# Weepingchestnut/SAVSR

Hardware: NVIDIA B200
Metric: hr_mpix_per_s (higher is better)
Workload: dtype bf16

## Files before the change

savsr_b200/csrc/conv_igemm.cu:

```cuda
#include <cstdio>
#include <cstdlib>

#include "common.cuh"

namespace savsr {

#ifdef SAVSR_DEBUG_COUNTERS
#define DBG_CLOCK() clock64()
#define DBG_ONLY(...) __VA_ARGS__
#else
#define DBG_CLOCK() 0ll
#define DBG_ONLY(...)
#endif

constexpr int kMaxAStages = 4;
constexpr int kHaloPitch = 10;
constexpr int kHaloStageBytes = 23552;
constexpr int kARegionBytes = 3 * kHaloStageBytes;
constexpr int kBBlocks = 18;
constexpr int kRing = 3;
constexpr int kEpiWarps = 8;
constexpr int kNumThreads = 64 + 32 * kEpiWarps;

struct ConvParams {
// ... 70 lines not shown
    if (c.res1_slot >= 0 && c.valid) {
      const uint4* r = reinterpret_cast<const uint4*>(p.arena + ((static_cast<long>(c.res1_slot) * p.batch + n) * npix + c.pix) * kC + col0);
#pragma unroll
      for (int j = 0; j < NC / 8; ++j) c.r1[j] = r[j];
    }
    if (c.res2_slot >= 0 && c.valid) {
      const uint4* r = reinterpret_cast<const uint4*>(p.arena + ((static_cast<long>(c.res2_slot) * p.batch + n) * npix + c.pix) * kC + col0);
#pragma unroll
      for (int j = 0; j < NC / 8; ++j) c.r2[j] = r[j];
    }
  }
}

__device__ __forceinline__ void add_h16x8(float* v, const uint4& u, float s, int fmt) {
  v[0] += s * h_lo(u.x, fmt); v[1] += s * h_hi(u.x, fmt); v[2] += s * h_lo(u.y, fmt); v[3] += s * h_hi(u.y, fmt);
  v[4] += s * h_lo(u.z, fmt); v[5] += s * h_hi(u.z, fmt); v[6] += s * h_lo(u.w, fmt); v[7] += s * h_hi(u.w, fmt);
}

template <int NC>
__device__ __forceinline__ void epi_finish(const ConvParams& p, const savsr_conv_group& g, int n, int tile, int quad, int lane,
                                           float (&v)[NC], int col0, const EpiCtx<NC>& c) {
  const long npix = static_cast<long>(p.height) * p.width;
  const float ns = c.neg_slope;
#pragma unroll
  for (int j = 0; j < NC; ++j) {
    const float t = v[j] + c.bias[j];
    v[j] = fmaxf(t, ns * t);
  }
  if constexpr (NC == 32) {
    if (c.has_mask) {
#pragma unroll
      for (int j = 0; j < NC; ++j) v[j] *= c.mk;
    }
    if (c.res1_slot >= 0 && c.valid) {
#pragma unroll
      for (int j = 0; j < NC / 8; ++j) add_h16x8(v + 8 * j, c.r1[j], 1.f, p.fmt);
    }
    if (c.res2_slot >= 0 && c.valid) {
      const float r2s = c.res2_scale;
#pragma unroll
      for (int j = 0; j < NC / 8; ++j) add_h16x8(v + 8 * j, c.r2[j], r2s, p.fmt);
    }
    if (c.valid) {
      uint4* d = reinterpret_cast<uint4*>(p.arena + ((static_cast<long>(c.dst_slot) * p.batch + n) * npix + c.pix) * kC + col0);
#pragma unroll
      for (int j = 0; j < NC / 8; ++j) {
        uint4 u;
        u.x = pack_h2(v[8 * j + 0], v[8 * j + 1], p.fmt);
        u.y = pack_h2(v[8 * j + 2], v[8 * j + 3], p.fmt);
        u.z = pack_h2(v[8 * j + 4], v[8 * j + 5], p.fmt);
        u.w = pack_h2(v[8 * j + 6], v[8 * j + 7], p.fmt);
        d[j] = u;
      }
    }
    if (c.pool != nullptr) {
      if (!c.valid) {
#pragma unroll
        for (int j = 0; j < NC; ++j) v[j] = 0.f;
      }
#pragma unroll
      for (int off = 16, cnt = 16; off >= 1; off >>= 1, cnt >>= 1) {
        const bool upper = (lane & off) != 0;
#pragma unroll
        for (int i = 0; i < cnt; ++i) {
          const float send = upper ? v[i] : v[i + cnt];
          const float keep = upper ? v[i + cnt] : v[i];
          v[i] = keep + __shfl_xor_sync(0xffffffffu, send, off);
        }
      }
      const int npart = p.tiles_x * p.tiles_y * 4;
      c.pool[(static_cast<long>(n) * npart + tile * 4 + quad) * kC + col0 + lane] = v[0];
    }
  } else {
    if (c.valid) {
      float4* d = reinterpret_cast<float4*>(static_cast<float*>(g.aux_dst) + (n * npix + c.pix) * 16);
#pragma unroll
      for (int j = 0; j < 4; ++j) d[j] = make_float4(v[4 * j], v[4 * j + 1], v[4 * j + 2], v[4 * j + 3]);
    }
  }
}


struct EpiQuad {
  float bias[8];
  uint4 r1[4], r2[4];
  float mk[4];
  long pix0;
  uint32_t valid;
  int bias_group;
  float neg_slope, res2_scale;
  int res1_slot, res2_slot, dst_slot;
  bool has_mask;
  float* pool;
  float psum[8];
};

__device__ __forceinline__ void epiq_prefetch(const ConvParams& p, const savsr_conv_group& g, int gi, int n, int tile, int quad,
                                              int lane, int half, EpiQuad& c) {
  const int tx = tile % p.tiles_x, ty = tile / p.tiles_x;
  const int px = tx * kTileW + (lane >> 2);
  const int py0 = ty * kTileH + quad * 4;
  const int rows = p.height - py0;
  c.valid = (px < p.width && rows > 0) ? (rows >= 4 ? 0xfu : ((1u << rows) - 1u)) : 0u;
  const long npix = static_cast<long>(p.height) * p.width;
  c.pix0 = static_cast<long>(py0) * p.width + px;
  const int ch0 = half * 32 + (lane & 3) * 8;
  if (gi != c.bias_group) {
    c.bias_group = gi;
    c.neg_slope = g.act == SAVSR_ACT_NONE ? 1.f : (g.act == SAVSR_ACT_RELU ? 0.f : g.slope);
    c.res2_scale = g.res2_scale;
    c.res1_slot = g.res1_slot; c.res2_slot = g.res2_slot; c.dst_slot = g.dst_slot;
    c.has_mask = g.mask != nullptr;
    c.pool = g.pool;
    if (g.bias != nullptr) {
      const float4 b0 = __ldg(reinterpret_cast<const float4*>(g.bias + ch0));
      const float4 b1 = __ldg(reinterpret_cast<const float4*>(g.bias + ch0) + 1);
      c.bias[0] = b0.x; c.bias[1] = b0.y; c.bias[2] = b0.z; c.bias[3] = b0.w;
      c.bias[4] = b1.x; c.bias[5] = b1.y; c.bias[6] = b1.z; c.bias[7] = b1.w;
    } else {
#pragma unroll
      for (int j = 0; j < 8; ++j) c.bias[j] = 0.f;
    }
  }
  if (c.has_mask) {
#pragma unroll
    for (int j = 0; j < 4; ++j) c.mk[j] = ((c.valid >> j) & 1u) ? __ldg(g.mask + n * npix + c.pix0 + j * p.width) : 0.f;
  }
  if (c.res1_slot >= 0) {
    const __nv_bfloat16* r = p.arena + ((static_cast<long>(c.res1_slot) * p.batch + n) * npix + c.pix0) * kC + ch0;
#pragma unroll
    for (int j = 0; j < 4; ++j)
      if ((c.valid >> j) & 1u) c.r1[j] = *reinterpret_cast<const uint4*>(r + static_cast<long>(j) * p.width * kC);
  }
  if (c.res2_slot >= 0) {
    const __nv_bfloat16* r = p.arena + ((static_cast<long>(c.res2_slot) * p.batch + n) * npix + c.pix0) * kC + ch0;
#pragma unroll
    for (int j = 0; j < 4; ++j)
      if ((c.valid >> j) & 1u) c.r2[j] = *reinterpret_cast<const uint4*>(r + static_cast<long>(j) * p.width * kC);
  }
}

template <class Release, class Next>
__device__ __forceinline__ void epiq_finish(const ConvParams& p, int n, int tile, int quad, int lane, int half, uint32_t taddr,
                                            EpiQuad& c, bool last_of_run, Release release, Next next) {
  uint32_t ra[16], rb[16];
  tmem_ld_16x256b_x4(taddr, ra);
  tmem_ld_16x256b_x4(taddr + (16u << 16), rb);
  tmem_ld_wait();
  tc_fence_before();
  __syncwarp();
  release();
  float v[4][8];
#pragma unroll
  for (int k = 0; k < 4; ++k) {
#pragma unroll
    for (int e = 0; e < 4; ++e) {
      v[e >> 1][2 * k + (e & 1)] = __uint_as_float(ra[4 * k + e]);
      v[2 + (e >> 1)][2 * k + (e & 1)] = __uint_as_float(rb[4 * k + e]);
    }
  }
  const long npix = static_cast<long>(p.height) * p.width;
  const int ch0 = half * 32 + (lane & 3) * 8;
  const float ns = c.neg_slope;
#pragma unroll
  for (int j = 0; j < 4; ++j) {
#pragma unroll
    for (int i = 0; i < 8; ++i) {
      const float t = v[j][i] + c.bias[i];
      v[j][i] = fmaxf(t, ns * t);
    }
  }
  if (c.has_mask) {
#pragma unroll
    for (int j = 0; j < 4; ++j) {
#pragma unroll
      for (int i = 0; i < 8; ++i) v[j][i] *= c.mk[j];
    }
  }
  if (c.res1_slot >= 0) {
#pragma unroll
    for (int j = 0; j < 4; ++j)
      if ((c.valid >> j) & 1u) add_h16x8(v[j], c.r1[j], 1.f, p.fmt);
  }
  if (c.res2_slot >= 0) {
    const float r2s = c.res2_scale;
#pragma unroll
    for (int j = 0; j < 4; ++j)
      if ((c.valid >> j) & 1u) add_h16x8(v[j], c.r2[j], r2s, p.fmt);
  }
  const uint32_t valid = c.valid;
  float* const pool = c.pool;
  __nv_bfloat16* d = p.arena + ((static_cast<long>(c.dst_slot) * p.batch + n) * npix + c.pix0) * kC + ch0;
  next();
#pragma unroll
  for (int j = 0; j < 4; ++j) {
    if ((valid >> j) & 1u) {
      uint4 u;
      u.x = pack_h2(v[j][0], v[j][1], p.fmt);
      u.y = pack_h2(v[j][2], v[j][3], p.fmt);
      u.z = pack_h2(v[j][4], v[j][5], p.fmt);
      u.w = pack_h2(v[j][6], v[j][7], p.fmt);
      *reinterpret_cast<uint4*>(d + static_cast<long>(j) * p.width * kC) = u;
    }
  }
  if (pool != nullptr) {
    if (valid == 0xfu) {
#pragma unroll
      for (int i = 0; i < 8; ++i) c.psum[i] += (v[0][i] + v[1][i]) + (v[2][i] + v[3][i]);
    } else {
#pragma unroll
      for (int i = 0; i < 8; ++i) {
        const float a0 = (valid & 1u) ? v[0][i] : 0.f, a1 = (valid & 2u) ? v[1][i] : 0.f;
        const float a2 = (valid & 4u) ? v[2][i] : 0.f, a3 = (valid & 8u) ? v[3][i] : 0.f;
        c.psum[i] += (a0 + a1) + (a2 + a3);
      }
    }
    const int npart = p.tiles_x * p.tiles_y * 4;
    const int ch = ch0 + ((lane >> 4) & 1) * 4 + ((lane >> 3) & 1) * 2 + ((lane >> 2) & 1);
    float total = 0.f;
    if (last_of_run) {
      float s[8];
#pragma unroll
      for (int i = 0; i < 8; ++i) { s[i] = c.psum[i]; c.psum[i] = 0.f; }
#pragma unroll
      for (int off = 16, cnt = 4; off >= 4; off >>= 1, cnt >>= 1) {
        const bool upper = (lane & off) != 0;
#pragma unroll
        for (int i = 0; i < cnt; ++i) {
          const float send = upper ? s[i] : s[i + cnt];
          const float keep = upper ? s[i + cnt] : s[i];
          s[i] = keep + __shfl_xor_sync(0xffffffffu, send, off);
        }
      }
      total = s[0];
    }
    pool[(static_cast<long>(n) * npart + tile * 4 + quad) * kC + ch] = total;
  }
}

__device__ __forceinline__ constexpr uint32_t desc_hi(uint32_t sbo_bytes) { return (sbo_bytes >> 4) | (1u << 14) | (2u << 29); }
__device__ __forceinline__ uint64_t make_desc(uint32_t hi, uint32_t lo) { return (static_cast<uint64_t>(hi) << 32) | lo; }

template <int BN, int KS, bool HALO>
__global__ void __launch_bounds__(kNumThreads, 1) conv_igemm_kernel(const __grid_constant__ ConvParams p) {
  constexpr int NT = KS * KS;
  extern __shared__ uint8_t smem_raw[];
  uint8_t* smem = reinterpret_cast<uint8_t*>((reinterpret_cast<uintptr_t>(smem_raw) + 1023) & ~static_cast<uintptr_t>(1023));
  constexpr int kBBytes = BN * 128;
  constexpr int kAStage = HALO ? kHaloStageBytes : kTileM * 128;
  constexpr int kAStages = HALO ? 3 : 4;
  uint8_t* smem_a = smem;
  uint8_t* smem_b = smem + kARegionBytes;
  uint8_t* smem_ring = smem_b + (kBBlocks - kRing) * kBBytes;
  uint64_t* bars = reinterpret_cast<uint64_t*>(smem_b + kBBlocks * kBBytes);
  uint64_t* a_full = bars;
  uint64_t* a_empty = a_full + kMaxAStages;
  uint64_t* res_full = a_empty + kMaxAStages;
  uint64_t* ring_full = res_full + kBBlocks;
  uint64_t* ring_empty = ring_full + kRing;
  uint64_t* res_free = ring_empty + kRing;
  uint64_t* t_full = res_free + 1;
  uint64_t* t_empty = t_full + 2;
  uint32_t* tmem_slot = reinterpret_cast<uint32_t*>(t_empty + 2);

  const int warp = threadIdx.x >> 5;
  const int lane = threadIdx.x & 31;
  const int tiles = p.tiles_x * p.tiles_y;
  const int total = p.ngroups * p.batch * tiles;
  const int item_begin = blockIdx.x * p.chunk;
  const int item_end = min(item_begin + p.chunk, total);
  const int nsrc = p.nsrc;
  const int n_res = p.n_res;
  constexpr int kTmemCols = 2 * BN < 32 ? 32 : 2 * BN;
  constexpr int kEpiArrivals = BN == 64 ? 8 : 4;

  if (warp == 0 && lane == 0) {
    prefetch_tensormap(HALO ? &p.tm_halo : &p.tm_tile);
    for (int i = 0; i < kMaxAStages; ++i) { mbar_init(a_full + i, 1); mbar_init(a_empty + i, 1); }
    for (int i = 0; i < kBBlocks; ++i) mbar_init(res_full + i, 1);
    for (int i = 0; i < kRing; ++i) { mbar_init(ring_full + i, 1); mbar_init(ring_empty + i, 1); }
    mbar_init(res_free, 1);
    for (int i = 0; i < 2; ++i) { mbar_init(t_full + i, 1); mbar_init(t_empty + i, kEpiArrivals); }
    fence_barrier_init();
  }
  if (warp == 1) tmem_alloc<kTmemCols>(tmem_slot);
  tc_fence_before();
  __syncthreads();
  tc_fence_after();
  const uint32_t tmem_base = *tmem_slot;

  if (warp == 0) {
    if (lane == 0) {
      int sa = 0, pa = 0, sr = 0, pr = 0;
      int gen = -1, cur_key = -1;
      long long dbg_ae = 0;
      const int nkb = nsrc * NT;
      int tile = item_begin % tiles;
      int gn = item_begin / tiles;
      for (int item = item_begin; item < item_end; ++item) {
        const int n = gn % p.batch;
        const int gi = gn / p.batch;
        const savsr_conv_group& g = p.g[gi];
        const int ty = tile / p.tiles_x;
        const int x0 = (tile - ty * p.tiles_x) * kTileW, y0 = ty * kTileH;
        const uint8_t* wptr = static_cast<const uint8_t*>(g.weight) + static_cast<long>(n) * g.weight_sample_stride;
        const int key = gi * p.batch + (g.weight_sample_stride != 0 ? n : 0);
        if (key != cur_key) {
          if (gen >= 0) mbar_wait(res_free, gen & 1);
          ++gen;
          cur_key = key;
          int kb = blockIdx.x % nkb;
          for (int i = 0; i < nkb; ++i) {
            if (kb < n_res) {
              mbar_expect_tx(res_full + kb, kBBytes);
              bulk_load(smem_b + kb * kBBytes, wptr + static_cast<long>(kb) * kBBytes, kBBytes, res_full + kb);
            }
            if (++kb == nkb) kb = 0;
          }
        }
        for (int s = 0; s < nsrc; ++s) {
// ... 79 lines not shown
#pragma unroll
              for (int k = 0; k < 4; ++k)
                umma_bf16(d_tmem, make_desc(a_hi, al + 2 * k), make_desc(b_hi, bl + 2 * k), idesc, (s | tap | k) ? 1u : 0u);
            }
            umma_commit(a_empty + sa);
          }
          __syncwarp();
          b_lo += NT * (kBBytes >> 4);
          if (++sa == kAStages) { sa = 0; pa ^= 1; }
        }
      } else {
        uint32_t accumulate = 0;
        uint32_t b_lo = b_lo0;
        int kb = 0;
        for (int s = 0; s < nsrc; ++s) {
          if constexpr (HALO) {
            mbar_wait(a_full + sa, pa);
            tc_fence_after();
          }
#pragma unroll
          for (int tap = 0; tap < NT; ++tap, ++kb, b_lo += kBBytes >> 4) {
            if constexpr (!HALO) {
              mbar_wait(a_full + sa, pa);
              tc_fence_after();
            }
            uint32_t bl = b_lo;
            const bool streamed = kb >= n_res;
            if (streamed) {
              mbar_wait(ring_full + sr, pr);
              tc_fence_after();
              bl = ring_lo0 + sr * (kBBytes >> 4);
            } else if (fresh) {
              mbar_wait(res_full + kb, gen & 1);
              tc_fence_after();
            }
            const uint32_t al = a_lo0 + sa * (kAStage >> 4) + (HALO ? ((tap / 3) * kHaloPitch + tap % 3) * 8 : 0);
            if (elect_one()) {
#pragma unroll
              for (int k = 0; k < 4; ++k) {
                umma_bf16(d_tmem, make_desc(a_hi, al + 2 * k), make_desc(b_hi, bl + 2 * k), idesc, accumulate);
                accumulate = 1;
              }
              if (streamed) umma_commit(ring_empty + sr);
              if (!HALO) umma_commit(a_empty + sa);
            }
            __syncwarp();
            accumulate = 1;
            if (streamed) {
              if (++sr == kRing) { sr = 0; pr ^= 1; }
            }
            if constexpr (!HALO) {
              if (++sa == kAStages) { sa = 0; pa ^= 1; }
            }
          }
          if constexpr (HALO) {
            if (elect_one()) umma_commit(a_empty + sa);
            __syncwarp();
            if (++sa == kAStages) { sa = 0; pa ^= 1; }
          }
        }
      }
      if (elect_one()) umma_commit(t_full + acc);
      __syncwarp();
      if (++tile == tiles) {
        tile = 0;
        if (++n == batch) { n = 0; ++gi; }
      }
    }
    DBG_ONLY(if (p.dbg != nullptr && lane == 0) {
      p.dbg[blockIdx.x * 8 + 0] = DBG_CLOCK() - dbg_t0;
      p.dbg[blockIdx.x * 8 + 1] = dbg_te;
      p.dbg[blockIdx.x * 8 + 2] = dbg_af;
      p.dbg[blockIdx.x * 8 + 3] = item_end - item_begin;
    })
    (void)dbg_te; (void)dbg_af; (void)dbg_t0;
  } else {
    const int quad = warp & 3;
    const int half = (warp - 2) >> 2;
    if (BN == 64 || half == 0) {
      constexpr int NC = 16;
      EpiCtx<NC> ec;
      EpiQuad eq;
      ec.bias_group = -1;
      eq.bias_group = -1;
#pragma unroll
      for (int i = 0; i < 8; ++i) eq.psum[i] = 0.f;
      int it = 0;
      int tile = item_begin % tiles;
      int gn = item_begin / tiles;
      long long dbg_tf = 0, dbg_t0 = DBG_CLOCK();
      if constexpr (BN == 64) {
        if (item_begin < item_end) epiq_prefetch(p, p.g[gn / p.batch], gn / p.batch, gn % p.batch, tile, quad, lane, half, eq);
      }
      for (int item = item_begin; item < item_end; ++item, ++it) {
        const int n = gn % p.batch;
        const int gi = gn / p.batch;
        const savsr_conv_group& g = p.g[gi];
        const int acc = it & 1;
        if constexpr (BN != 64) epi_prefetch<NC>(p, g, gi, n, tile, quad, lane, 0, ec);
        const long long c0 = DBG_CLOCK();
        mbar_wait(t_full + acc, (it >> 1) & 1);
        dbg_tf += DBG_CLOCK() - c0;
        tc_fence_after();
        const uint32_t taddr = tmem_base + (static_cast<uint32_t>(quad * 32) << 16) + static_cast<uint32_t>(acc * BN + half * 32);
        if constexpr (BN == 64) {
          epiq_finish(p, n, tile, quad, lane, half, taddr, eq, item + 1 >= item_end || tile + 1 == tiles,
                      [&] { if (lane == 0) mbar_arrive(t_empty + acc); }, [&] {
            if (item + 1 < item_end) {
              const int nt = tile + 1 == tiles ? 0 : tile + 1, ngn = tile + 1 == tiles ? gn + 1 : gn;
              epiq_prefetch(p, p.g[ngn / p.batch], ngn / p.batch, ngn % p.batch, nt, quad, lane, half, eq);
            }
          });
        } else {
          float v[NC];
          uint32_t r[16];
          tmem_ld16(taddr, r);
          tmem_ld_wait();
#pragma unroll
          for (int c = 0; c < 16; ++c) v[c] = __uint_as_float(r[c]);
          tc_fence_before();
          __syncwarp();
          if (lane == 0) mbar_arrive(t_empty + acc);
          epi_finish<NC>(p, g, n, tile, quad, lane, v, 0, ec);
        }
        if (++tile == tiles) { tile = 0; ++gn; }
      }
      DBG_ONLY(if (p.dbg != nullptr && warp == 2 && lane == 0) {
        p.dbg[blockIdx.x * 8 + 4] = DBG_CLOCK() - dbg_t0;
        p.dbg[blockIdx.x * 8 + 5] = dbg_tf;
      })
      (void)dbg_tf; (void)dbg_t0;
    }
  }

  tc_fence_before();
  __syncthreads();
  if (warp == 1) {
    tc_fence_after();
    tmem_dealloc<kTmemCols>(tmem_base);
  }
}

constexpr int kBatchTiles = 4;

constexpr int kBigkThreads = kNumThreads + 32;

__global__ void __launch_bounds__(kBigkThreads, 1) conv_igemm_bigk_kernel(const __grid_constant__ ConvParams p) {
  constexpr int BN = 64, NT = 9;
  constexpr int kBBytes = BN * 128;
  constexpr int kAStage = kHaloStageBytes, kAStages = 3;
  constexpr int kSetBlocks = 9, kSetBytes = kSetBlocks * kBBytes;
  extern __shared__ uint8_t smem_raw[];
  uint8_t* smem = reinterpret_cast<uint8_t*>((reinterpret_cast<uintptr_t>(smem_raw) + 1023) & ~static_cast<uintptr_t>(1023));
  uint8_t* smem_a = smem;
  uint8_t* smem_b = smem + kARegionBytes;
  uint64_t* bars = reinterpret_cast<uint64_t*>(smem_b + 2 * kSetBytes);
  uint64_t* a_full = bars;
  uint64_t* a_empty = a_full + kMaxAStages;
  uint64_t* set_full = a_empty + kMaxAStages;
  uint64_t* set_empty = set_full + 2;
  uint64_t* t_full = set_empty + 2;
  uint64_t* t_empty = t_full + 2 * kBatchTiles;
  uint32_t* tmem_slot = reinterpret_cast<uint32_t*>(t_empty + 2 * kBatchTiles);

  const int warp = threadIdx.x >> 5;
  const int lane = threadIdx.x & 31;
  const int tiles = p.tiles_x * p.tiles_y;
  const int total = p.ngroups * p.batch * tiles;
  const int item_begin = blockIdx.x * p.chunk;
  const int item_end = min(item_begin + p.chunk, total);
  const int nsrc = p.nsrc;
  const bool pinned = nsrc <= 2;
  const uint32_t ps_mask = p.per_sample_mask;

  if (warp == 0 && lane == 0) {
    prefetch_tensormap(&p.tm_halo);
    for (int i = 0; i < kMaxAStages; ++i) { mbar_init(a_full + i, 1); mbar_init(a_empty + i, p.issuers); }
    for (int i = 0; i < 2; ++i) { mbar_init(set_full + i, 1); mbar_init(set_empty + i, p.issuers); }
    for (int i = 0; i < 2 * kBatchTiles; ++i) { mbar_init(t_full + i, 1); mbar_init(t_empty + i, 8); }
    fence_barrier_init();
  }
  if (warp == 1) tmem_alloc<512>(tmem_slot);
  tc_fence_before();
  __syncthreads();
  tc_fence_after();
  const uint32_t tmem_base = *tmem_slot;
  pdl_wait();
  pdl_trigger();

  int item = item_begin;
  int tile = item_begin % tiles;
  int gn = item_begin / tiles;
  int bcount = 0;
  uint32_t use_bits = 0;
  uint32_t set_loads[2] = {0, 0};
  int cur_key = -1;

  if (warp == 0) {
    if (lane == 0) {
      int sa = 0, pa = 0;
      uint32_t u = 0;
      while (item < item_end) {
        const int cnt = min(kBatchTiles, min(item_end - item, tiles - tile));
        const int n = gn % p.batch;
        const int gi = gn / p.batch;
        const savsr_conv_group& g = p.g[gi];
        const uint8_t* wptr = static_cast<const uint8_t*>(g.weight) + static_cast<long>(n) * g.weight_sample_stride;
        const int key = gi * p.batch + (((ps_mask >> gi) & 1u) ? n : 0);
        const bool load = !pinned || key != cur_key;
        cur_key = key;
        for (int s = 0; s < nsrc; ++s) {
          if (load) {
            const int set = pinned ? s : static_cast<int>(u++ & 1);
            mbar_wait(set_empty + set, (set_loads[set] & 1u) ^ 1u);
            ++set_loads[set];
            mbar_expect_tx(set_full + set, kSetBytes);
            int kb = blockIdx.x % kSetBlocks;
            for (int i = 0; i < kSetBlocks; ++i) {
              bulk_load(smem_b + set * kSetBytes + kb * kBBytes, wptr + static_cast<long>(s * NT + kb) * kBBytes, kBBytes, set_full + set);
              if (++kb == kSetBlocks) kb = 0;
            }
          }
          const int img = g.src_slot[s] * p.batch + n;
          for (int j = 0; j < cnt; ++j) {
            const int tj = tile + j;
            const int ty = tj / p.tiles_x;
            mbar_wait(a_empty + sa, pa ^ 1);
            mbar_expect_tx(a_full + sa, kHaloPitch * (kTileH + 2) * 128u);
            tma_load_4d(smem_a + sa * kAStage, &p.tm_halo, a_full + sa, 0, (tj - ty * p.tiles_x) * kTileW - 1, ty * kTileH - 1, img);
            if (++sa == kAStages) { sa = 0; pa ^= 1; }
          }
        }
        item += cnt; tile += cnt;
        if (tile == tiles) { tile = 0; ++gn; }
      }
    }
  } else if (warp == 1 || (warp == 10 && p.issuers == 2)) {
    const int my = warp == 1 ? 0 : 1;
    const int own_mask = p.issuers == 2 ? 1 : 0;
    const uint32_t idesc = umma_idesc_f16(BN, p.fmt);
    constexpr uint32_t a_hi = desc_hi(kHaloPitch * 128u);
    constexpr uint32_t b_hi = desc_hi(1024u);
    const uint32_t a_lo0 = (smem_u32(smem_a) >> 4) & 0x3fffu;
    const uint32_t b_lo0 = (smem_u32(smem_b) >> 4) & 0x3fffu;
    int sa = 0, pa = 0;
    uint32_t u = 0;
    long long dbg_te = 0, dbg_af = 0, dbg_sf = 0, dbg_t0 = DBG_CLOCK(), c0;
    while (item < item_end) {
      const int cnt = min(kBatchTiles, min(item_end - item, tiles - tile));
      const int bb = bcount & 1;
      const int n = gn % p.batch;
      const int gi = gn / p.batch;
      const int key = gi * p.batch + (((ps_mask >> gi) & 1u) ? n : 0);
      const bool load = !pinned || key != cur_key;
      if (pinned && load && cur_key >= 0) {
        if (elect_one()) {
          for (int s = 0; s < nsrc; ++s) umma_commit(set_empty + s);
        }
        __syncwarp();
      }
      cur_key = key;
      c0 = DBG_CLOCK();
#pragma unroll
      for (int j = 0; j < kBatchTiles; ++j) {
// ... 4 lines not shown
      for (int s = 0; s < nsrc; ++s) {
        const int set = pinned ? s : static_cast<int>(u & 1);
        if (load) {
          c0 = DBG_CLOCK();
          mbar_wait(set_full + set, set_loads[set] & 1u);
          dbg_sf += DBG_CLOCK() - c0;
          ++set_loads[set];
          tc_fence_after();
          ++u;
        }
        const uint32_t bl0 = b_lo0 + set * (kSetBytes >> 4);
#pragma unroll
        for (int j = 0; j < kBatchTiles; ++j) {
          if (j < cnt) {
            c0 = DBG_CLOCK();
            mbar_wait(a_full + sa, pa);
            dbg_af += DBG_CLOCK() - c0;
            if ((j & own_mask) != my) {
              if (elect_one()) mbar_arrive(a_empty + sa);
              __syncwarp();
            } else {
              tc_fence_after();
              const uint32_t al0 = a_lo0 + sa * (kAStage >> 4);
              const uint32_t d_tmem = tmem_base + static_cast<uint32_t>((bb * kBatchTiles + j) * BN);
              if (elect_one()) {
                uint32_t al = al0, bl = bl0, acc = s ? 1u : 0u;
                if (p.ksteps == 4) {
#pragma unroll 1
                  for (int dy = 0; dy < 3; ++dy) {
#pragma unroll
                    for (int dx = 0; dx < 3; ++dx) {
#pragma unroll
                      for (int k = 0; k < 4; ++k) {
                        umma_bf16(d_tmem, make_desc(a_hi, al + dx * 8 + 2 * k), make_desc(b_hi, bl + dx * (kBBytes >> 4) + 2 * k), idesc, acc);
                        acc = 1u;
                      }
                    }
                    al += kHaloPitch * 8;
                    bl += 3 * (kBBytes >> 4);
                  }
                } else {
#pragma unroll 1
                  for (int dy = 0; dy < 3; ++dy) {
#pragma unroll
                    for (int dx = 0; dx < 3; ++dx) {
#pragma unroll 1
                      for (int k = 0; k < p.ksteps; ++k) {
                        umma_bf16(d_tmem, make_desc(a_hi, al + dx * 8 + 2 * k), make_desc(b_hi, bl + dx * (kBBytes >> 4) + 2 * k), idesc, acc);
                        acc = 1u;
                      }
                    }
                    al += kHaloPitch * 8;
                    bl += 3 * (kBBytes >> 4);
                  }
                }
                umma_commit(a_empty + sa);
                if (s == nsrc - 1) umma_commit(t_full + bb * kBatchTiles + j);
              }
              __syncwarp();
            }
            if (++sa == kAStages) { sa = 0; pa ^= 1; }
          }
        }
        if (!pinned) {
          if (elect_one()) umma_commit(set_empty + set);
          __syncwarp();
        }
      }
#pragma unroll
      for (int j = 0; j < kBatchTiles; ++j)
        if (j < cnt) use_bits ^= 1u << (bb * kBatchTiles + j);
      ++bcount;
      item += cnt; tile += cnt;
      if (tile == tiles) { tile = 0; ++gn; }
    }
    DBG_ONLY(if (p.dbg != nullptr && lane == 0 && my == 0) {
      p.dbg[blockIdx.x * 8 + 0] = DBG_CLOCK() - dbg_t0;
      p.dbg[blockIdx.x * 8 + 1] = dbg_te;
      p.dbg[blockIdx.x * 8 + 2] = dbg_af;
      p.dbg[blockIdx.x * 8 + 3] = item_end - item_begin;
      p.dbg[blockIdx.x * 8 + 7] = dbg_sf;
    })
    (void)dbg_te; (void)dbg_af; (void)dbg_sf; (void)dbg_t0;
  } else if (warp < 10) {
    const int quad = warp & 3;
    const int half = (warp - 2) >> 2;
    EpiQuad eq;
    eq.bias_group = -1;
#pragma unroll
    for (int i = 0; i < 8; ++i) eq.psum[i] = 0.f;
    long long dbg_tf = 0, dbg_t0 = DBG_CLOCK();
    if (item < item_end) epiq_prefetch(p, p.g[gn / p.batch], gn / p.batch, gn % p.batch, tile, quad, lane, half, eq);
    while (item < item_end) {
      const int cnt = min(kBatchTiles, min(item_end - item, tiles - tile));
      const int bb = bcount & 1;
      const int n = gn % p.batch;
      for (int j = 0; j < cnt; ++j) {
        const int acc = bb * kBatchTiles + j;
        const long long c0 = DBG_CLOCK();
        mbar_wait(t_full + acc, (use_bits >> acc) & 1u);
        dbg_tf += DBG_CLOCK() - c0;
        use_bits ^= 1u << acc;
        tc_fence_after();
        const uint32_t taddr = tmem_base + (static_cast<uint32_t>(quad * 32) << 16) + static_cast<uint32_t>(acc * BN + half * 32);
        epiq_finish(p, n, tile + j, quad, lane, half, taddr, eq, item + j + 1 >= item_end || tile + j + 1 == tiles,
                    [&] { if (lane == 0) mbar_arrive(t_empty + acc); }, [&] {
          if (item + j + 1 < item_end) {
            const int nt = tile + j + 1 == tiles ? 0 : tile + j + 1, ngn = tile + j + 1 == tiles ? gn + 1 : gn;
            epiq_prefetch(p, p.g[ngn / p.batch], ngn / p.batch, ngn % p.batch, nt, quad, lane, half, eq);
          }
        });
      }
      ++bcount;
      item += cnt; tile += cnt;
      if (tile == tiles) { tile = 0; ++gn; }
    }
    DBG_ONLY(if (p.dbg != nullptr && warp == 2 && lane == 0) {
      p.dbg[blockIdx.x * 8 + 4] = DBG_CLOCK() - dbg_t0;
      p.dbg[blockIdx.x * 8 + 5] = dbg_tf;
    })
    (void)dbg_tf; (void)dbg_t0;
  }

  tc_fence_before();
  __syncthreads();
  if (warp == 1) {
    tc_fence_after();
    tmem_dealloc<512>(tmem_base);
  }
}

template <int BN>
__global__ void __launch_bounds__(128) conv_check_kernel(const __grid_constant__ ConvParams p) {
  const int tiles = p.tiles_x * p.tiles_y;
  const int item = blockIdx.x;
  const int tile = item % tiles;
  const int gn = item / tiles;
  const int n = gn % p.batch;
  const int gi = gn / p.batch;
  const savsr_conv_group& g = p.g[gi];
  const int m = threadIdx.x;
  const int px = (tile % p.tiles_x) * kTileW + (m & 7);
  const int py = (tile / p.tiles_x) * kTileH + (m >> 3);
  const long npix = static_cast<long>(p.height) * p.width;
  const uint8_t* wptr = static_cast<const uint8_t*>(g.weight) + static_cast<long>(n) * g.weight_sample_stride;
  constexpr int NC = BN == 64 ? 32 : 16;
  for (int col0 = 0; col0 < BN; col0 += NC) {
    float v[NC];
#pragma unroll
    for (int c = 0; c < NC; ++c) v[c] = 0.f;
    for (int s = 0; s < g.nsrc; ++s) {
      const __nv_bfloat16* src = p.arena + (static_cast<long>(g.src_slot[s]) * p.batch + n) * npix * kC;
      for (int tap = 0; tap < p.ntaps; ++tap) {
        const int dx = p.ntaps == 9 ? tap % 3 - 1 : 0, dy = p.ntaps == 9 ? tap / 3 - 1 : 0;
        const int sx = px + dx, sy = py + dy;
        const bool in = sx >= 0 && sx < p.width && sy >= 0 && sy < p.height;
        const uint8_t* wb = wptr + static_cast<long>(s * p.ntaps + tap) * (BN * 128);
        for (int k = 0; k < 64; ++k) {
          const float a = in ? h_to_float(reinterpret_cast<const uint16_t*>(src)[(static_cast<long>(sy) * p.width + sx) * kC + k], p.fmt) : 0.f;
#pragma unroll
          for (int c = 0; c < NC; ++c) {
            const int row = BN == 64 ? quad_row(col0 + c) : col0 + c;
            const int off = row * 128 + (((k >> 3) ^ (row & 7)) << 4) + (k & 7) * 2;
            v[c] += a * h_to_float(*reinterpret_cast<const uint16_t*>(wb + off), p.fmt);
          }
        }
      }
    }
    EpiCtx<NC> ec;
    ec.bias_group = -1;
    epi_prefetch<NC>(p, g, gi, n, tile, m >> 5, m & 31, col0, ec);
    epi_finish<NC>(p, g, n, tile, m >> 5, m & 31, v, col0, ec);
  }
}

__global__ void pack_weight_kernel(const float* __restrict__ w, int co_real, int co, int ci, int ks, int n_tile, int fmt, int quad,
                                   uint16_t* __restrict__ out) {
  const long total = static_cast<long>(co) * ci * ks * ks;
  const int taps = ks * ks;
  for (long idx = blockIdx.x * static_cast<long>(blockDim.x) + threadIdx.x; idx < total;
       idx += static_cast<long>(gridDim.x) * blockDim.x) {
    const int k = idx & 63;
    long r = idx >> 6;
    const int n = r % n_tile; r /= n_tile;
    const int kb = r % ((ci / 64) * taps);
    const int ng = r / ((ci / 64) * taps);
    const int s = kb / taps, tap = kb % taps;
    const int o = ng * n_tile + (quad ? quad_row(n) : n), i = s * 64 + k;
    const float val = o < co_real ? w[(static_cast<long>(o) * ci + i) * taps + tap] : 0.f;
    const long block = static_cast<long>(ng) * ((ci / 64) * taps) + kb;
    const long off = block * (n_tile * 64) + n * 64 + ((((k >> 3) ^ (n & 7)) << 3) | (k & 7));
    out[off] = float_to_h(val, fmt);
  }
}

__global__ void arena_import_kernel(const float* __restrict__ nchw, uint16_t* __restrict__ dst, int batch, long npix, int fmt) {
  const long total = static_cast<long>(batch) * npix * kC;
  for (long idx = blockIdx.x * static_cast<long>(blockDim.x) + threadIdx.x; idx < total;
       idx += static_cast<long>(gridDim.x) * blockDim.x) {
    const int c = idx & 63;
    const long pn = idx >> 6;
    const long pix = pn % npix, n = pn / npix;
    dst[idx] = float_to_h(nchw[(n * kC + c) * npix + pix], fmt);
  }
}
__global__ void arena_export_kernel(const uint16_t* __restrict__ src, float* __restrict__ nchw, int batch, long npix, int fmt) {
  const long total = static_cast<long>(batch) * npix * kC;
  for (long idx = blockIdx.x * static_cast<long>(blockDim.x) + threadIdx.x; idx < total;
       idx += static_cast<long>(gridDim.x) * blockDim.x) {
    const long pix = idx % npix;
    const long nc = idx / npix;
    const int c = nc % kC;
    const long n = nc / kC;
    nchw[idx] = h_to_float(src[(n * npix + pix) * kC + c], fmt);
  }
}

template <int BN, int KS, bool HALO>
static int launch_igemm(savsr_ctx* ctx, ConvParams& p, int total, cudaStream_t st) {
  const size_t smem = 1024 + kARegionBytes + kBBlocks * BN * 128 + 512;
  constexpr int variant = (BN == 64 ? 0 : 3) + (KS == 1 ? 0 : (HALO ? 1 : 2));
  if (int rc = ensure_smem_attr(ctx, kAttrIgemm + variant, conv_igemm_kernel<BN, KS, HALO>, smem)) return rc;
  p.chunk = (total + ctx->sm_count - 1) / ctx->sm_count;
  const int grid = (total + p.chunk - 1) / p.chunk;
  conv_igemm_kernel<BN, KS, HALO><<<grid, kNumThreads, smem, st>>>(p);
  SAVSR_CUDA(cudaGetLastError());
  return 0;
}

template <int BN>
static int launch_conv(savsr_ctx* ctx, ConvParams& p, int impl, cudaStream_t st) {
  const int total = p.ngroups * p.batch * p.tiles_x * p.tiles_y;
  if (total == 0) return 0;
  if (impl == SAVSR_IMPL_CHECK) {
    conv_check_kernel<BN><<<total, 128, 0, st>>>(p);
    SAVSR_CUDA(cudaGetLastError());
    return 0;
  }
  if (p.ntaps == 1) return launch_igemm<BN, 1, false>(ctx, p, total, st);
  if constexpr (BN == 64) {
    if (p.halo && (ctx->opt[SAVSR_OPT_BIGK_ALL] || p.nsrc * p.ntaps > kBBlocks)) {
      const size_t smem = 1024 + kARegionBytes + kBBlocks * BN * 128 + 512;
      if (int rc = ensure_smem_attr(ctx, kAttrBigk, conv_igemm_bigk_kernel, smem)) return rc;
      p.chunk = (total + ctx->sm_count - 1) / ctx->sm_count;
      const int grid = (total + p.chunk - 1) / p.chunk;
      SAVSR_CUDA(launch_k(ctx->opt[SAVSR_OPT_PDL] != 0, conv_igemm_bigk_kernel, dim3(grid), dim3(kBigkThreads), smem, st, p));
      return 0;
    }
  }
  if (p.halo) return launch_igemm<BN, 3, true>(ctx, p, total, st);
  return launch_igemm<BN, 3, false>(ctx, p, total, st);
}

}

using namespace savsr;

#ifdef SAVSR_DEBUG_COUNTERS
extern "C" void savsr_debug_conv_counters(savsr_ctx* ctx, long long* dev_buf) { if (ctx) ctx->conv_dbg = dev_buf; }
#endif

extern "C" size_t savsr_packed_weight_bytes(int co, int ci, int ksize) {
  return static_cast<size_t>(co) * ci * ksize * ksize * sizeof(__nv_bfloat16);
}

extern "C" int savsr_pack_conv_weight(const float* w_oihw, int co_real, int co, int ci, int ksize, int n_tile, int format,
                                      int row_order, void* packed, savsr_stream st) {
  SAVSR_REQUIRE(format == SAVSR_FMT_BF16 || format == SAVSR_FMT_FP16, "savsr_pack_conv_weight: unknown format %d", format);
  SAVSR_REQUIRE(row_order == SAVSR_ROWS_LINEAR || row_order == SAVSR_ROWS_QUAD, "savsr_pack_conv_weight: unknown row_order %d", row_order);
  SAVSR_REQUIRE(w_oihw && packed, "savsr_pack_conv_weight: null pointer");
  SAVSR_REQUIRE(ksize == 1 || ksize == 3, "savsr_pack_conv_weight: ksize must be 1 or 3, got %d", ksize);
  SAVSR_REQUIRE(n_tile == 64 || n_tile == 16, "savsr_pack_conv_weight: n_tile must be 64 or 16, got %d", n_tile);
  SAVSR_REQUIRE(ci > 0 && ci % 64 == 0, "savsr_pack_conv_weight: ci (%d) must be a positive multiple of 64", ci);
  SAVSR_REQUIRE(co > 0 && co % n_tile == 0 && co_real <= co && co_real > 0,
                "savsr_pack_conv_weight: co (%d) must be a multiple of n_tile (%d) and >= co_real (%d)", co, n_tile, co_real);
  const long total = static_cast<long>(co) * ci * ksize * ksize;
  const int blocks = static_cast<int>((total + 255) / 256 < 2048 ? (total + 255) / 256 : 2048);
  pack_weight_kernel<<<blocks, 256, 0, static_cast<cudaStream_t>(st)>>>(w_oihw, co_real, co, ci, ksize, n_tile, format,
                                                                       (n_tile == 64 && row_order == SAVSR_ROWS_QUAD) ? 1 : 0,
                                                                       static_cast<uint16_t*>(packed));
  SAVSR_CUDA(cudaGetLastError());
  return 0;
}

extern "C" int savsr_arena_import(savsr_arena* a, int slot, const float* nchw, savsr_stream st) {
  SAVSR_REQUIRE(a && nchw, "savsr_arena_import: null pointer");
  SAVSR_REQUIRE(slot >= 0 && slot < a->nslots, "savsr_arena_import: slot %d out of range [0,%d)", slot, a->nslots);
  const long npix = static_cast<long>(a->height) * a->width;
  arena_import_kernel<<<1024, 256, 0, static_cast<cudaStream_t>(st)>>>(
      nchw, reinterpret_cast<uint16_t*>(a->base + static_cast<long>(slot) * a->batch * npix * kC), a->batch, npix, a->ctx->fmt);
  SAVSR_CUDA(cudaGetLastError());
  return 0;
}

extern "C" int savsr_arena_export(savsr_arena* a, int slot, float* nchw, savsr_stream st) {
  SAVSR_REQUIRE(a && nchw, "savsr_arena_export: null pointer");
  SAVSR_REQUIRE(slot >= 0 && slot < a->nslots, "savsr_arena_export: slot %d out of range [0,%d)", slot, a->nslots);
  const long npix = static_cast<long>(a->height) * a->width;
  arena_export_kernel<<<1024, 256, 0, static_cast<cudaStream_t>(st)>>>(
      reinterpret_cast<const uint16_t*>(a->base + static_cast<long>(slot) * a->batch * npix * kC), nchw, a->batch, npix, a->ctx->fmt);
  SAVSR_CUDA(cudaGetLastError());
  return 0;
}

extern "C" int savsr_conv(savsr_ctx* ctx, savsr_arena* arena, const savsr_conv_group* groups, int ngroups, int ksize,
                          int n_tile, int dst_mode, int impl, savsr_stream st) {
  SAVSR_REQUIRE(ctx && arena && groups, "savsr_conv: null pointer");
  DeviceGuard guard(ctx->device);
  SAVSR_REQUIRE(ngroups >= 0 && ngroups <= SAVSR_MAX_GROUPS, "savsr_conv: ngroups %d out of range [0,%d]", ngroups, SAVSR_MAX_GROUPS);
  SAVSR_REQUIRE(ksize == 1 || ksize == 3, "savsr_conv: ksize must be 1 or 3, got %d", ksize);
  SAVSR_REQUIRE(impl >= SAVSR_IMPL_TCGEN05_TAP && impl <= SAVSR_IMPL_CHECK, "savsr_conv: unknown impl %d", impl);
  SAVSR_REQUIRE((n_tile == 64 && dst_mode == SAVSR_DST_ARENA) || (n_tile == 16 && dst_mode == SAVSR_DST_AUX16),
                "savsr_conv: n_tile %d does not match dst_mode %d", n_tile, dst_mode);
  if (ngroups == 0) return 0;

  ConvParams p;
  memset(&p, 0, sizeof(p));
  p.tm_tile = arena->tm_tile;
  p.tm_halo = arena->tm_halo;
  for (int i = 0; i < ngroups; ++i) {
    const savsr_conv_group& g = groups[i];
    SAVSR_REQUIRE(g.nsrc >= 1 && g.nsrc <= SAVSR_MAX_SRC, "savsr_conv: group %d nsrc %d out of range", i, g.nsrc);
    SAVSR_REQUIRE(g.weight != nullptr, "savsr_conv: group %d has no weights", i);
    SAVSR_REQUIRE(g.nsrc == groups[0].nsrc, "savsr_conv: all groups of a launch must have the same nsrc (%d vs %d)", g.nsrc, groups[0].nsrc);
    SAVSR_REQUIRE(g.src_channels == groups[0].src_channels && g.src_channels >= 0 && g.src_channels <= 64 && g.src_channels % 16 == 0,
// ... 36 lines not shown
```

Measured before the change: 270.3.

## Double epilogue warps in big-K conv kernel with alternating tile ownership

The big-K conv kernel now runs 16 epilogue warps in two groups that take alternate accumulator tiles, so the TMEM drain and store epilogue keeps pace with the MMA issuer. Pool running sums move into shared memory, with an mbarrier handoff between the groups to keep per-run channel sums in order. The epilogue also loads TMEM in two halves and reads group parameters directly rather than caching them, which lowers register pressure. The cost is more threads, extra shared memory, and cross-group synchronisation when pooling is active.

```diff
diff --git a/savsr_b200/csrc/conv_igemm.cu b/savsr_b200/csrc/conv_igemm.cu
--- a/savsr_b200/csrc/conv_igemm.cu
+++ b/savsr_b200/csrc/conv_igemm.cu
@@ -176,160 +176,153 @@
 
 
 struct EpiQuad {
-  float bias[8];
   uint4 r1[4], r2[4];
   float mk[4];
   long pix0;
   uint32_t valid;
-  int bias_group;
-  float neg_slope, res2_scale;
-  int res1_slot, res2_slot, dst_slot;
-  bool has_mask;
-  float* pool;
-  float psum[8];
+  int gi;
 };
 
-__device__ __forceinline__ void epiq_prefetch(const ConvParams& p, const savsr_conv_group& g, int gi, int n, int tile, int quad,
-                                              int lane, int half, EpiQuad& c) {
+__device__ __forceinline__ void epiq_prefetch(const ConvParams& p, int gi, int n, int tile, int quad, int lane, int half, EpiQuad& c) {
+  const savsr_conv_group& g = p.g[gi];
   const int tx = tile % p.tiles_x, ty = tile / p.tiles_x;
   const int px = tx * kTileW + (lane >> 2);
   const int py0 = ty * kTileH + quad * 4;
   const int rows = p.height - py0;
+  c.gi = gi;
   c.valid = (px < p.width && rows > 0) ? (rows >= 4 ? 0xfu : ((1u << rows) - 1u)) : 0u;
   const long npix = static_cast<long>(p.height) * p.width;
   c.pix0 = static_cast<long>(py0) * p.width + px;
   const int ch0 = half * 32 + (lane & 3) * 8;
-  if (gi != c.bias_group) {
-    c.bias_group = gi;
-    c.neg_slope = g.act == SAVSR_ACT_NONE ? 1.f : (g.act == SAVSR_ACT_RELU ? 0.f : g.slope);
-    c.res2_scale = g.res2_scale;
-    c.res1_slot = g.res1_slot; c.res2_slot = g.res2_slot; c.dst_slot = g.dst_slot;
-    c.has_mask = g.mask != nullptr;
-    c.pool = g.pool;
-    if (g.bias != nullptr) {
-      const float4 b0 = __ldg(reinterpret_cast<const float4*>(g.bias + ch0));
-      const float4 b1 = __ldg(reinterpret_cast<const float4*>(g.bias + ch0) + 1);
-      c.bias[0] = b0.x; c.bias[1] = b0.y; c.bias[2] = b0.z; c.bias[3] = b0.w;
-      c.bias[4] = b1.x; c.bias[5] = b1.y; c.bias[6] = b1.z; c.bias[7] = b1.w;
-    } else {
-#pragma unroll
-      for (int j = 0; j < 8; ++j) c.bias[j] = 0.f;
-    }
-  }
-  if (c.has_mask) {
+  if (g.mask != nullptr) {
 #pragma unroll
     for (int j = 0; j < 4; ++j) c.mk[j] = ((c.valid >> j) & 1u) ? __ldg(g.mask + n * npix + c.pix0 + j * p.width) : 0.f;
   }
-  if (c.res1_slot >= 0) {
-    const __nv_bfloat16* r = p.arena + ((static_cast<long>(c.res1_slot) * p.batch + n) * npix + c.pix0) * kC + ch0;
+  if (g.res1_slot >= 0) {
+    const __nv_bfloat16* r = p.arena + ((static_cast<long>(g.res1_slot) * p.batch + n) * npix + c.pix0) * kC + ch0;
 #pragma unroll
     for (int j = 0; j < 4; ++j)
       if ((c.valid >> j) & 1u) c.r1[j] = *reinterpret_cast<const uint4*>(r + static_cast<long>(j) * p.width * kC);
   }
-  if (c.res2_slot >= 0) {
-    const __nv_bfloat16* r = p.arena + ((static_cast<long>(c.res2_slot) * p.batch + n) * npix + c.pix0) * kC + ch0;
+  if (g.res2_slot >= 0) {
+    const __nv_bfloat16* r = p.arena + ((static_cast<long>(g.res2_slot) * p.batch + n) * npix + c.pix0) * kC + ch0;
 #pragma unroll
     for (int j = 0; j < 4; ++j)
       if ((c.valid >> j) & 1u) c.r2[j] = *reinterpret_cast<const uint4*>(r + static_cast<long>(j) * p.width * kC);
   }
 }
 
-template <class Release, class Next>
-__device__ __forceinline__ void epiq_finish(const ConvParams& p, int n, int tile, int quad, int lane, int half, uint32_t taddr,
-                                            EpiQuad& c, bool last_of_run, Release release, Next next) {
-  uint32_t ra[16], rb[16];
-  tmem_ld_16x256b_x4(taddr, ra);
-  tmem_ld_16x256b_x4(taddr + (16u << 16), rb);
-  tmem_ld_wait();
-  tc_fence_before();
-  __syncwarp();
-  release();
-  float v[4][8];
-#pragma unroll
-  for (int k = 0; k < 4; ++k) {
-#pragma unroll
-    for (int e = 0; e < 4; ++e) {
-      v[e >> 1][2 * k + (e & 1)] = __uint_as_float(ra[4 * k + e]);
-      v[2 + (e >> 1)][2 * k + (e & 1)] = __uint_as_float(rb[4 * k + e]);
-    }
+template <class Release>
+__device__ __forceinline__ float* epiq_finish(const ConvParams& p, int n, int quad, int lane, int half, uint32_t taddr,
+                                              const EpiQuad& c, float (&tsum)[8], Release release) {
+  const savsr_conv_group& g = p.g[c.gi];
+  const int ch0 = half * 32 + (lane & 3) * 8;
+  float bias[8];
+  if (g.bias != nullptr) {
+    const float4 b0 = __ldg(reinterpret_cast<const float4*>(g.bias + ch0));
+    const float4 b1 = __ldg(reinterpret_cast<const float4*>(g.bias + ch0) + 1);
+    bias[0] = b0.x; bias[1] = b0.y; bias[2] = b0.z; bias[3] = b0.w;
+    bias[4] = b1.x; bias[5] = b1.y; bias[6] = b1.z; bias[7] = b1.w;
+  } else {
+#pragma unroll
+    for (int j = 0; j < 8; ++j) bias[j] = 0.f;
   }
   const long npix = static_cast<long>(p.height) * p.width;
-  const int ch0 = half * 32 + (lane & 3) * 8;
-  const float ns = c.neg_slope;
-#pragma unroll
-  for (int j = 0; j < 4; ++j) {
-#pragma unroll
-    for (int i = 0; i < 8; ++i) {
-      const float t = v[j][i] + c.bias[i];
-      v[j][i] = fmaxf(t, ns * t);
-    }
-  }
-  if (c.has_mask) {
-#pragma unroll
-    for (int j = 0; j < 4; ++j) {
-#pragma unroll
-      for (int i = 0; i < 8; ++i) v[j][i] *= c.mk[j];
-    }
-  }
-  if (c.res1_slot >= 0) {
-#pragma unroll
-    for (int j = 0; j < 4; ++j)
-      if ((c.valid >> j) & 1u) add_h16x8(v[j], c.r1[j], 1.f, p.fmt);
-  }
-  if (c.res2_slot >= 0) {
-    const float r2s = c.res2_scale;
-#pragma unroll
-    for (int j = 0; j < 4; ++j)
-      if ((c.valid >> j) & 1u) add_h16x8(v[j], c.r2[j], r2s, p.fmt);
-  }
+  const float ns = g.act == SAVSR_ACT_NONE ? 1.f : (g.act == SAVSR_ACT_RELU ? 0.f : g.slope);
   const uint32_t valid = c.valid;
-  float* const pool = c.pool;
-  __nv_bfloat16* d = p.arena + ((static_cast<long>(c.dst_slot) * p.batch + n) * npix + c.pix0) * kC + ch0;
-  next();
-#pragma unroll
-  for (int j = 0; j < 4; ++j) {
-    if ((valid >> j) & 1u) {
-      uint4 u;
-      u.x = pack_h2(v[j][0], v[j][1], p.fmt);
-      u.y = pack_h2(v[j][2], v[j][3], p.fmt);
-      u.z = pack_h2(v[j][4], v[j][5], p.fmt);
-      u.w = pack_h2(v[j][6], v[j][7], p.fmt);
-      *reinterpret_cast<uint4*>(d + static_cast<long>(j) * p.width * kC) = u;
-    }
-  }
-  if (pool != nullptr) {
-    if (valid == 0xfu) {
-#pragma unroll
-      for (int i = 0; i < 8; ++i) c.psum[i] += (v[0][i] + v[1][i]) + (v[2][i] + v[3][i]);
-    } else {
+  float* const pool = g.pool;
+  __nv_bfloat16* d = p.arena + ((static_cast<long>(g.dst_slot) * p.batch + n) * npix + c.pix0) * kC + ch0;
+#pragma unroll
+  for (int hp = 0; hp < 2; ++hp) {
+    uint32_t r[16];
+    tmem_ld_16x256b_x4(taddr + (static_cast<uint32_t>(16 * hp) << 16), r);
+    tmem_ld_wait();
+    if (hp == 1) {
+      tc_fence_before();
+      __syncwarp();
+      release();
+    }
+    float v[2][8];
+#pragma unroll
+    for (int k = 0; k < 4; ++k) {
+#pragma unroll
+      for (int e = 0; e < 4; ++e) v[e >> 1][2 * k + (e & 1)] = __uint_as_float(r[4 * k + e]);
+    }
+#pragma unroll
+    for (int jj = 0; jj < 2; ++jj) {
 #pragma unroll
       for (int i = 0; i < 8; ++i) {
-        const float a0 = (valid & 1u) ? v[0][i] : 0.f, a1 = (valid & 2u) ? v[1][i] : 0.f;
-        const float a2 = (valid & 4u) ? v[2][i] : 0.f, a3 = (valid & 8u) ? v[3][i] : 0.f;
-        c.psum[i] += (a0 + a1) + (a2 + a3);
-      }
-    }
-    const int npart = p.tiles_x * p.tiles_y * 4;
-    const int ch = ch0 + ((lane >> 4) & 1) * 4 + ((lane >> 3) & 1) * 2 + ((lane >> 2) & 1);
-    float total = 0.f;
-    if (last_of_run) {
-      float s[8];
-#pragma unroll
-      for (int i = 0; i < 8; ++i) { s[i] = c.psum[i]; c.psum[i] = 0.f; }
-#pragma unroll
-      for (int off = 16, cnt = 4; off >= 4; off >>= 1, cnt >>= 1) {
-        const bool upper = (lane & off) != 0;
-#pragma unroll
-        for (int i = 0; i < cnt; ++i) {
-          const float send = upper ? s[i] : s[i + cnt];
-          const float keep = upper ? s[i + cnt] : s[i];
-          s[i] = keep + __shfl_xor_sync(0xffffffffu, send, off);
-        }
-      }
-      total = s[0];
-    }
-    pool[(static_cast<long>(n) * npart + tile * 4 + quad) * kC + ch] = total;
-  }
+        const float t = v[jj][i] + bias[i];
+        v[jj][i] = fmaxf(t, ns * t);
+      }
+    }
+    if (g.mask != nullptr) {
+#pragma unroll
+      for (int jj = 0; jj < 2; ++jj) {
+#pragma unroll
+        for (int i = 0; i < 8; ++i) v[jj][i] *= c.mk[2 * hp + jj];
+      }
+    }
+    if (g.res1_slot >= 0) {
+#pragma unroll
+      for (int jj = 0; jj < 2; ++jj)
+        if ((valid >> (2 * hp + jj)) & 1u) add_h16x8(v[jj], c.r1[2 * hp + jj], 1.f, p.fmt);
+    }
+    if (g.res2_slot >= 0) {
+      const float r2s = g.res2_scale;
+#pragma unroll
+      for (int jj = 0; jj < 2; ++jj)
+        if ((valid >> (2 * hp + jj)) & 1u) add_h16x8(v[jj], c.r2[2 * hp + jj], r2s, p.fmt);
+    }
+#pragma unroll
+    for (int jj = 0; jj < 2; ++jj) {
+      if ((valid >> (2 * hp + jj)) & 1u) {
+        uint4 u;
+        u.x = pack_h2(v[jj][0], v[jj][1], p.fmt);
+        u.y = pack_h2(v[jj][2], v[jj][3], p.fmt);
+        u.z = pack_h2(v[jj][4], v[jj][5], p.fmt);
+        u.w = pack_h2(v[jj][6], v[jj][7], p.fmt);
+        *reinterpret_cast<uint4*>(d + static_cast<long>(2 * hp + jj) * p.width * kC) = u;
+      }
+    }
+    if (pool != nullptr) {
+      if (valid == 0xfu) {
+#pragma unroll
+        for (int i = 0; i < 8; ++i) tsum[i] = hp == 0 ? v[0][i] + v[1][i] : tsum[i] + (v[0][i] + v[1][i]);
+      } else {
+#pragma unroll
+        for (int i = 0; i < 8; ++i) {
+          const float a0 = ((valid >> (2 * hp)) & 1u) ? v[0][i] : 0.f, a1 = ((valid >> (2 * hp + 1)) & 1u) ? v[1][i] : 0.f;
+          tsum[i] = hp == 0 ? a0 + a1 : tsum[i] + (a0 + a1);
+        }
+      }
+    }
+  }
+  return pool;
+}
+
+__device__ __forceinline__ void epiq_pool_store(const ConvParams& p, float* pool, int n, int tile, int quad, int lane, int half,
+                                                float (&run)[8], bool last_of_run) {
+  const int npart = p.tiles_x * p.tiles_y * 4;
+  const int ch = half * 32 + (lane & 3) * 8 + ((lane >> 4) & 1) * 4 + ((lane >> 3) & 1) * 2 + ((lane >> 2) & 1);
+  float total = 0.f;
+  if (last_of_run) {
+    float s[8];
+#pragma unroll
+    for (int i = 0; i < 8; ++i) { s[i] = run[i]; run[i] = 0.f; }
+#pragma unroll
+    for (int off = 16, cnt = 4; off >= 4; off >>= 1, cnt >>= 1) {
+      const bool upper = (lane & off) != 0;
+#pragma unroll
+      for (int i = 0; i < cnt; ++i) {
+        const float send = upper ? s[i] : s[i + cnt];
+        const float keep = upper ? s[i + cnt] : s[i];
+        s[i] = keep + __shfl_xor_sync(0xffffffffu, send, off);
+      }
+    }
+    total = s[0];
+  }
+  pool[(static_cast<long>(n) * npart + tile * 4 + quad) * kC + ch] = total;
 }
 
 __device__ __forceinline__ constexpr uint32_t desc_hi(uint32_t sbo_bytes) { return (sbo_bytes >> 4) | (1u << 14) | (2u << 29); }
@@ -575,15 +568,15 @@
       EpiCtx<NC> ec;
       EpiQuad eq;
       ec.bias_group = -1;
-      eq.bias_group = -1;
-#pragma unroll
-      for (int i = 0; i < 8; ++i) eq.psum[i] = 0.f;
+      float psum[8];
+#pragma unroll
+      for (int i = 0; i < 8; ++i) psum[i] = 0.f;
       int it = 0;
       int tile = item_begin % tiles;
       int gn = item_begin / tiles;
       long long dbg_tf = 0, dbg_t0 = DBG_CLOCK();
       if constexpr (BN == 64) {
-        if (item_begin < item_end) epiq_prefetch(p, p.g[gn / p.batch], gn / p.batch, gn % p.batch, tile, quad, lane, half, eq);
+        if (item_begin < item_end) epiq_prefetch(p, gn / p.batch, gn % p.batch, tile, quad, lane, half, eq);
       }
       for (int item = item_begin; item < item_end; ++item, ++it) {
         const int n = gn % p.batch;
@@ -597,13 +590,17 @@
         tc_fence_after();
         const uint32_t taddr = tmem_base + (static_cast<uint32_t>(quad * 32) << 16) + static_cast<uint32_t>(acc * BN + half * 32);
         if constexpr (BN == 64) {
-          epiq_finish(p, n, tile, quad, lane, half, taddr, eq, item + 1 >= item_end || tile + 1 == tiles,
-                      [&] { if (lane == 0) mbar_arrive(t_empty + acc); }, [&] {
-            if (item + 1 < item_end) {
-              const int nt = tile + 1 == tiles ? 0 : tile + 1, ngn = tile + 1 == tiles ? gn + 1 : gn;
-              epiq_prefetch(p, p.g[ngn / p.batch], ngn / p.batch, ngn % p.batch, nt, quad, lane, half, eq);
-            }
-          });
+          float tsum[8];
+          float* pool = epiq_finish(p, n, quad, lane, half, taddr, eq, tsum, [&] { if (lane == 0) mbar_arrive(t_empty + acc); });
+          if (pool != nullptr) {
+#pragma unroll
+            for (int i = 0; i < 8; ++i) psum[i] += tsum[i];
+            epiq_pool_store(p, pool, n, tile, quad, lane, half, psum, item + 1 >= item_end || tile + 1 == tiles);
+          }
+          if (item + 1 < item_end) {
+            const int nt = tile + 1 == tiles ? 0 : tile + 1, ngn = tile + 1 == tiles ? gn + 1 : gn;
+            epiq_prefetch(p, ngn / p.batch, ngn % p.batch, nt, quad, lane, half, eq);
+          }
         } else {
           float v[NC];
           uint32_t r[16];
@@ -635,8 +632,9 @@
 }
 
 constexpr int kBatchTiles = 4;
-
-constexpr int kBigkThreads = kNumThreads + 32;
+constexpr int kBigkEpiWarps = 16;
+constexpr int kBigkThreads = 64 + 32 * kBigkEpiWarps + 32;
+constexpr int kRunSumBytes = 8 * 32 * 8 * 4;
 
 __global__ void __launch_bounds__(kBigkThreads, 1) conv_igemm_bigk_kernel(const __grid_constant__ ConvParams p) {
   constexpr int BN = 64, NT = 9;
@@ -654,7 +652,9 @@
   uint64_t* set_empty = set_full + 2;
   uint64_t* t_full = set_empty + 2;
   uint64_t* t_empty = t_full + 2 * kBatchTiles;
-  uint32_t* tmem_slot = reinterpret_cast<uint32_t*>(t_empty + 2 * kBatchTiles);
+  uint64_t* run_full = t_empty + 2 * kBatchTiles;
+  uint32_t* tmem_slot = reinterpret_cast<uint32_t*>(run_full + 8);
+  float4* run_sums = reinterpret_cast<float4*>(reinterpret_cast<uint8_t*>(bars) + 512);
 
   const int warp = threadIdx.x >> 5;
   const int lane = threadIdx.x & 31;
@@ -671,8 +671,10 @@
     for (int i = 0; i < kMaxAStages; ++i) { mbar_init(a_full + i, 1); mbar_init(a_empty + i, p.issuers); }
     for (int i = 0; i < 2; ++i) { mbar_init(set_full + i, 1); mbar_init(set_empty + i, p.issuers); }
     for (int i = 0; i < 2 * kBatchTiles; ++i) { mbar_init(t_full + i, 1); mbar_init(t_empty + i, 8); }
+    for (int i = 0; i < 8; ++i) mbar_init(run_full + i, 1);
     fence_barrier_init();
   }
+  for (int i = threadIdx.x; i < kRunSumBytes / 16; i += kBigkThreads) run_sums[i] = make_float4(0.f, 0.f, 0.f, 0.f);
   if (warp == 1) tmem_alloc<512>(tmem_slot);
   tc_fence_before();
   __syncthreads();
@@ -843,20 +845,42 @@
       p.dbg[blockIdx.x * 8 + 7] = dbg_sf;
     })
     (void)dbg_te; (void)dbg_af; (void)dbg_sf; (void)dbg_t0;
-  } else if (warp < 10) {
+  } else if (warp != 10) {
+    const int grp = warp < 10 ? 0 : 1;
     const int quad = warp & 3;
-    const int half = (warp - 2) >> 2;
+    const int half = (warp - (grp ? 11 : 2)) >> 2;
+    float4* const run = run_sums + (half * 4 + quad) * 64 + lane;
+    uint64_t* const run_bar = run_full + half * 4 + quad;
+    bool pooled = false;
+    for (int i = 0; i < p.ngroups; ++i) pooled |= p.g[i].pool != nullptr;
+    uint32_t handovers = 0;
+    int prev_owner = -1;
+    auto find_own = [&](int it, int t, int g, int j, int& ft, int& fg) {
+      while (it < item_end) {
+        const int c = min(kBatchTiles, min(item_end - it, tiles - t));
+        if (j < c) { ft = t + j; fg = g; return true; }
+        it += c; t += c;
+        if (t == tiles) { t = 0; ++g; }
+        j = grp;
+      }
+      return false;
+    };
     EpiQuad eq;
-    eq.bias_group = -1;
-#pragma unroll
-    for (int i = 0; i < 8; ++i) eq.psum[i] = 0.f;
     long long dbg_tf = 0, dbg_t0 = DBG_CLOCK();
-    if (item < item_end) epiq_prefetch(p, p.g[gn / p.batch], gn / p.batch, gn % p.batch, tile, quad, lane, half, eq);
+    int ft, fg;
+    if (find_own(item, tile, gn, grp, ft, fg)) epiq_prefetch(p, fg / p.batch, fg % p.batch, ft, quad, lane, half, eq);
     while (item < item_end) {
       const int cnt = min(kBatchTiles, min(item_end - item, tiles - tile));
       const int bb = bcount & 1;
       const int n = gn % p.batch;
       for (int j = 0; j < cnt; ++j) {
+        const int owner = j & 1;
+        const bool take = pooled && prev_owner >= 0 && prev_owner != owner;
+        const uint32_t h = handovers;
+        handovers += take ? 1u : 0u;
+        prev_owner = owner;
+        if (owner != grp) continue;
+        const bool give = pooled && (j + 1 < cnt || (owner == 1 && item + cnt < item_end));
         const int acc = bb * kBatchTiles + j;
         const long long c0 = DBG_CLOCK();
         mbar_wait(t_full + acc, (use_bits >> acc) & 1u);
@@ -864,13 +888,22 @@
         use_bits ^= 1u << acc;
         tc_fence_after();
         const uint32_t taddr = tmem_base + (static_cast<uint32_t>(quad * 32) << 16) + static_cast<uint32_t>(acc * BN + half * 32);
-        epiq_finish(p, n, tile + j, quad, lane, half, taddr, eq, item + j + 1 >= item_end || tile + j + 1 == tiles,
-                    [&] { if (lane == 0) mbar_arrive(t_empty + acc); }, [&] {
-          if (item + j + 1 < item_end) {
-            const int nt = tile + j + 1 == tiles ? 0 : tile + j + 1, ngn = tile + j + 1 == tiles ? gn + 1 : gn;
-            epiq_prefetch(p, p.g[ngn / p.batch], ngn / p.batch, ngn % p.batch, nt, quad, lane, half, eq);
-          }
-        });
+        float tsum[8];
+        float* const pool = epiq_finish(p, n, quad, lane, half, taddr, eq, tsum, [&] { if (lane == 0) mbar_arrive(t_empty + acc); });
+        if (take) mbar_wait(run_bar, h & 1u);
+        if (pool != nullptr) {
+          const float4 r0 = run[0], r1 = run[32];
+          float s[8] = {r0.x + tsum[0], r0.y + tsum[1], r0.z + tsum[2], r0.w + tsum[3],
+                        r1.x + tsum[4], r1.y + tsum[5], r1.z + tsum[6], r1.w + tsum[7]};
+          epiq_pool_store(p, pool, n, tile + j, quad, lane, half, s, item + j + 1 >= item_end || tile + j + 1 == tiles);
+          run[0] = make_float4(s[0], s[1], s[2], s[3]);
+          run[32] = make_float4(s[4], s[5], s[6], s[7]);
+        }
+        if (give) {
+          __syncwarp();
+          if (lane == 0) mbar_arrive(run_bar);
+        }
+        if (find_own(item, tile, gn, j + 2, ft, fg)) epiq_prefetch(p, fg / p.batch, fg % p.batch, ft, quad, lane, half, eq);
       }
       ++bcount;
       item += cnt; tile += cnt;
@@ -1001,7 +1034,7 @@
   if (p.ntaps == 1) return launch_igemm<BN, 1, false>(ctx, p, total, st);
   if constexpr (BN == 64) {
     if (p.halo && (ctx->opt[SAVSR_OPT_BIGK_ALL] || p.nsrc * p.ntaps > kBBlocks)) {
-      const size_t smem = 1024 + kARegionBytes + kBBlocks * BN * 128 + 512;
+      const size_t smem = 1024 + kARegionBytes + kBBlocks * BN * 128 + 512 + kRunSumBytes;
       if (int rc = ensure_smem_attr(ctx, kAttrBigk, conv_igemm_bigk_kernel, smem)) return rc;
       p.chunk = (total + ctx->sm_count - 1) / ctx->sm_count;
       const int grid = (total + p.chunk - 1) / p.chunk;
```

Result: slower. 199.5, median of 6 (-26.2%).
